# young-how/DQN-based-UAV-3D_path_planer

Hardware: NVIDIA H100
Metric: env steps/sec (+ DQN updates/sec), 500x500x100 city (higher is better)
Workload: dtype f64 env state / f32 obs+learner

## Files before the change

dqn-based-uav-3d_path_planer_b200/csrc/tc_forward.cu:

```cuda
#include "tc_forward.cuh"
#include "env_block.cuh"

#include <stdlib.h>
#include <string.h>

#include "tma.cuh"
#include "wgmma.cuh"

namespace uavrl {

static inline int rup(int x, int m) { return (x + m - 1) / m * m; }

size_t tc_smem_bytes(const TcNet &tc) { return (size_t)2 * tc.a_bytes + (size_t)tc.img_bytes + (size_t)tc.max_rows * tc.acc_ld * 4; }

int tc_build(const uavrl_learner_config &c, const NetDev &net, TcNet &tc, std::vector<int32_t> &hi_map, std::vector<int32_t> &lo_map,
             std::vector<int32_t> &hi2_map, std::vector<int32_t> &lo2_map)
{
    memset(&tc, 0, sizeof(tc));
    tc.n_layers = net.n_layers; tc.in_dim = net.in_dim; tc.n_actions = net.n_actions; tc.dueling = net.dueling;
    if (net.in_dim % 4 != 0) return -1;
    int off = 0, maxK = 0, k_pad = rup(net.in_dim, 8);
    for (int l = 0; l < net.n_layers; ++l) {
        const LayerDev &L = net.L[l];
        TcLayer &T = tc.L[l];
// ... 61 lines not shown
                if (l > 0) {
                    hi2_map[pi] = elem(T.N_pad, T.t_hi_off, k, o);
                    lo2_map[pi] = elem(T.N_pad, T.t_lo_off, k, o);
                }
            }
            hi_map[vrow ? (size_t)L.b2_off + (o - out_main) : (size_t)L.b_off + o] = tc.bias_base / 4 + T.bias_off + o;
        }
    }
    (void)c;
    return 0;
}


#define TC_TRACE(slot) do { if (a.trace && blockIdx.x == 0 && threadIdx.x == 0) a.trace[slot] = clock64(); } while (0)

template <bool FUSE_ENV, bool ACT, bool DUELING>
__global__ void __launch_bounds__(kTcThreads, 1) tc_forward_kernel_t(TcNet tc, TcArgs a, EnvFuse ef)
{
    TC_TRACE(0);
    extern __shared__ __align__(1024) unsigned char smem[];
    unsigned char *Ahi = smem, *Alo = smem + tc.a_bytes, *W = smem + 2 * tc.a_bytes;
    float *acc = reinterpret_cast<float *>(W + tc.img_bytes);
    __shared__ uint64_t wbar, wbar2;
    __shared__ const float *rows[kTcTile];
    __shared__ float s_rew[kTcTile], s_done[kTcTile];

    const int tid = threadIdx.x, warp = tid >> 5, lane = tid & 31, quad = warp & 3, half = warp >> 2;
    constexpr int kCtl = kTcThreads - 32;
    const bool early_w = (a.pdl & kPdlEarlyWeights) != 0;
    const uint32_t w_split = tc.n_layers > 1 ? (uint32_t)tc.L[1].hi_off : (uint32_t)tc.img_bytes;
    auto stage_image = [&]() {
// ... 72 lines not shown
            waited = true;
            if (tid == kCtl && !early_w) stage_image();
        }
        if (!wready) {
            __syncthreads();
            mbar_wait(&wbar, 0);
            wready = true;
        }
        TC_TRACE(3);
        fence_proxy_async();
        __syncthreads();
        TC_TRACE(4);

        for (int l = 0; l < tc.n_layers; ++l) {
            const TcLayer T = tc.L[l];
            mma_3xtf32(acc, tc.acc_ld, Ahi, Alo, W + T.hi_off, W + T.lo_off, mma_sbo(T.K_pad), T.N_pad, T.K_pad / 8, R);
            TC_TRACE(5 + 3 * l);
            if (!w2ready) { if (w_split < (uint32_t)tc.img_bytes) mbar_wait(&wbar2, 0); w2ready = true; }
            TC_TRACE(6 + 3 * l);
            const float *bias = bias_all + T.bias_off;
            const int row = quad * 32 + lane;
            const bool live = quad * 32 < R;
            if (l + 1 < tc.n_layers) {
                const uint32_t sbon = mma_sbo(T.N_pad);
                for (int c0 = half * 32; live && c0 < T.N_pad; c0 += 64) {
                    float v[32];
                    acc_ld32(acc, tc.acc_ld, row, c0, v);
#pragma unroll
                    for (int j = 0; j < 8; ++j) {
                        float4 h, lo4;
                        float x0 = fmaxf(v[4 * j + 0] + bias[c0 + 4 * j + 0], 0.f), x1 = fmaxf(v[4 * j + 1] + bias[c0 + 4 * j + 1], 0.f);
                        float x2 = fmaxf(v[4 * j + 2] + bias[c0 + 4 * j + 2], 0.f), x3 = fmaxf(v[4 * j + 3] + bias[c0 + 4 * j + 3], 0.f);
                        tf32_split(x0, h.x, lo4.x); tf32_split(x1, h.y, lo4.y); tf32_split(x2, h.z, lo4.z); tf32_split(x3, h.w, lo4.w);
                        const uint32_t off = mma_off(row, c0 + 4 * j, sbon);
                        *reinterpret_cast<float4 *>(Ahi + off) = h;
                        *reinterpret_cast<float4 *>(Alo + off) = lo4;
                    }
                }
                fence_proxy_async();
                __syncthreads();
                TC_TRACE(7 + 3 * l);
            } else {
                if (half == 0 && live) {
                    float q[32];
                    acc_ld32(acc, tc.acc_ld, row, 0, q);
                    const int nA = tc.n_actions;
#pragma unroll
                    for (int j = 0; j < 32; ++j) q[j] += bias[j];
                    if (DUELING) {
                        float s = 0.f;
#pragma unroll
                        for (int j = 0; j < 32; ++j) if (j < nA) s += q[j];
// ... 39 lines not shown
                }
                __syncthreads();
            }
        }
        if (FUSE_ENV) {
            __shared__ EnvSmem<32> env_sm;
            for (int sb = 0; sb < R; sb += 32)
                env_block<true, 32, kTcThreads, false, 8>(ef.d, env_sm, base + sb, tid, UAVRL_ACT_DISCRETE27, a.actions, ef.obs_next,
                                                       ef.reward, ef.done, nullptr, nullptr, nullptr);
            __syncthreads();
        }
    }
    TC_TRACE(20);
}

typedef void (*ForwardKernel)(TcNet, TcArgs, EnvFuse);
template <bool F, bool A>
static ForwardKernel pick_fwd_d(bool dueling) { return dueling ? tc_forward_kernel_t<F, A, true> : tc_forward_kernel_t<F, A, false>; }
static ForwardKernel pick_forward_kernel(bool fuse_env, bool act, bool dueling)
{
    if (fuse_env) return pick_fwd_d<true, true>(dueling);
    return act ? pick_fwd_d<false, true>(dueling) : pick_fwd_d<false, false>(dueling);
}

int launch_tc_forward(uavrl_learner *l, const TcArgs &a_in, cudaStream_t st, const EnvFuse *fuse)
{
    TcArgs a = a_in;
    const int n_sm = num_sms();
    a.rows_per_tile = (a.n >= 128 * n_sm && l->tc.max_rows == 128) ? 128 : (a.n >= 64 * n_sm) ? 64 : 32;
    a.n_tiles = (a.n + a.rows_per_tile - 1) / a.rows_per_tile;
    const int grid = a.n_tiles < n_sm ? a.n_tiles : n_sm;
    static const bool trace_on = getenv("UAVRL_TC_TRACE") != nullptr;
    long long *tr = nullptr;
    if (trace_on) { UAVRL_CUDA(cudaMalloc((void **)&tr, 32 * sizeof(long long))); UAVRL_CUDA(cudaMemset(tr, 0, 32 * sizeof(long long))); a.trace = tr; }
    const int prev = (l->pdl_chain && g_pdl.load()) ? l->pdl_prev : kPdlNone;
    a.pdl = 0;
    if (prev != kPdlNone) {
        a.pdl = kPdlOn;
        if (a.mode == kTcAct) {
            if (prev == kPdlAdam) a.pdl |= kPdlEarlyRows;
            else if (prev == kPdlEnv) a.pdl |= kPdlEarlyWeights;
        } else if (prev == kPdlEnv || prev == kPdlTd) {
            a.pdl |= kPdlEarlyWeights;
        }
    }
    EnvFuse ef;
    memset(&ef, 0, sizeof(ef));
    if (fuse) {
        ef = *fuse;
        UAVRL_CUDA(launch_kernel(pick_forward_kernel(true, a.mode == kTcAct, l->tc.dueling != 0), dim3(grid), dim3(kTcThreads), tc_smem_bytes(l->tc), st, a.pdl != 0, l->tc, a, ef));
        l->pdl_prev = l->pdl_chain ? kPdlEnv : kPdlNone;
    } else {
        UAVRL_CUDA(launch_kernel(pick_forward_kernel(false, a.mode == kTcAct, l->tc.dueling != 0), dim3(grid), dim3(kTcThreads), tc_smem_bytes(l->tc), st, a.pdl != 0, l->tc, a, ef));
        l->pdl_prev = l->pdl_chain ? (a.mode == kTcAct ? kPdlAct : kPdlTd) : kPdlNone;
    }
    UAVRL_LAUNCHED();
    if (trace_on) {
        long long h[32];
        UAVRL_CUDA(cudaStreamSynchronize(st));
        UAVRL_CUDA(cudaMemcpy(h, tr, sizeof(h), cudaMemcpyDeviceToHost));
        cudaFree(tr);
        fprintf(stderr, "[tc_trace] mode=%d n=%d R=%d grid=%d cycles since start:", a.mode, a.n, a.rows_per_tile, grid);
        for (int i = 1; i < 32; ++i) if (h[i]) fprintf(stderr, " [%d]=%lld", i, h[i] - h[0]);
        fprintf(stderr, "\n");
    }
    return 0;
}

// ... 5 lines not shown
    if (tc_smem_bytes(l->tc) > 227 * 1024) return 0;
    const size_t P = (size_t)l->net.P;
    const size_t img = (size_t)l->tc.train_img_bytes;
    UAVRL_CUDA(cudaMalloc((void **)&l->tc_img_local, img));
    UAVRL_CUDA(cudaMalloc((void **)&l->tc_img_target, img));
    UAVRL_CUDA(cudaMemset(l->tc_img_local, 0, img));
    UAVRL_CUDA(cudaMemset(l->tc_img_target, 0, img));
    int32_t **maps[] = { &l->tc_hi_map, &l->tc_lo_map, &l->tc_hi2_map, &l->tc_lo2_map };
    std::vector<int32_t> *src[] = { &hi, &lo, &hi2, &lo2 };
    for (int i = 0; i < 4; ++i) {
        UAVRL_CUDA(cudaMalloc((void **)maps[i], P * 4));
        UAVRL_CUDA(cudaMemcpy(*maps[i], src[i]->data(), P * 4, cudaMemcpyHostToDevice));
    }
    UAVRL_CUDA(cudaMalloc((void **)&l->y_buf, (size_t)l->cfg.batch_size * 4));
    UAVRL_CUDA(cudaMalloc((void **)&l->astar_buf, (size_t)l->cfg.batch_size * 4));
    for (int ac = 0; ac < 2; ++ac)
        for (int du = 0; du < 2; ++du)
            UAVRL_CUDA(cudaFuncSetAttribute(pick_forward_kernel(false, ac != 0, du != 0), cudaFuncAttributeMaxDynamicSharedMemorySize,
                                            (int)tc_smem_bytes(l->tc)));
    {
        l->fuse_ok = true;
        for (int du = 0; du < 2; ++du) {
            cudaFuncAttributes fa;
            UAVRL_CUDA(cudaFuncGetAttributes(&fa, pick_forward_kernel(true, true, du != 0)));
            if (fa.sharedSizeBytes + tc_smem_bytes(l->tc) > (size_t)227 * 1024) l->fuse_ok = false;
        }
        if (l->fuse_ok)
            for (int du = 0; du < 2; ++du)
                UAVRL_CUDA(cudaFuncSetAttribute(pick_forward_kernel(true, true, du != 0), cudaFuncAttributeMaxDynamicSharedMemorySize,
                                                (int)tc_smem_bytes(l->tc)));
    }
    l->y_cap = l->cfg.batch_size;
    l->tc_ok = true;
    return tc_train_init(l);
}

}
```

dqn-based-uav-3d_path_planer_b200/csrc/tc_forward.cuh:

```cuda
#pragma once
#include <vector>

#include "env.cuh"
#include "learner.cuh"

namespace uavrl {

constexpr int kTcThreads = 256;
constexpr int kTcTile = 128;

enum TcMode { kTcAct = 0, kTcArgmax = 1, kTcTdMax = 2, kTcTdGather = 3 };

struct TcArgs {
    const unsigned char *img;
    BatchSrc src;
    const float *obs;
    int32_t n, n_tiles, mode, use_next, rows_per_tile;
    float eps; int32_t is_train;
    const float *u_tape; const int32_t *rand_tape;
    uint64_t key, call;
    int32_t *actions;
    float *q_out;
    float *y_out;
    float gamma;
    int32_t pdl;
    long long *trace;
};

int tc_build(const uavrl_learner_config &c, const NetDev &net, TcNet &tc, std::vector<int32_t> &hi_map, std::vector<int32_t> &lo_map,
             std::vector<int32_t> &hi2_map, std::vector<int32_t> &lo2_map);
int tc_train_init(uavrl_learner *l);
int launch_tc_train(uavrl_learner *l, const BatchSrc &src, int B, int global_batch, const float *y, int *n_grad_parts,
                    int *n_loss_parts, cudaStream_t st, cudaEvent_t after_chain = nullptr, const AdamArgs *adam = nullptr,
                    float *loss_out = nullptr, bool *adam_done = nullptr, bool fused_td = false);
bool tc_train_can_fuse_td(const uavrl_learner *l, int B);
size_t tc_smem_bytes(const TcNet &tc);
struct EnvFuse { EnvDev d; float *obs_next; float *reward; uint8_t *done; };
int launch_tc_forward(uavrl_learner *l, const TcArgs &a, cudaStream_t st, const EnvFuse *fuse = nullptr);
int tc_init(uavrl_learner *l);

}
```

dqn-based-uav-3d_path_planer_b200/csrc/tc_train.cu:

```cuda
#include <string.h>
#include <stdlib.h>

#include <atomic>

#include "tc_forward.cuh"
#include "tma.cuh"
#include "wgmma.cuh"

namespace uavrl {

constexpr int kDwChunk = 128;

struct TcTrainArgs {
    const unsigned char *img;
    BatchSrc src;
    int32_t B, R, n_tiles;
    const float *y;
    float inv_global_b;
    float *act_buf, *dz_buf;
    float *loss_partials;
    int32_t loss_kind;
    int32_t fused_td, algo;
    float gamma;
    const unsigned char *img_target;
// ... 78 lines not shown
    for (int u = 0; u < 4; ++u) {
        const int i = threadIdx.x + u * kTcThreads;
        if (i < total) {
            const int r = i & (R - 1), j = i >> lgR;
            float4 h, l;
            tf32_split(v[u].x, h.x, l.x); tf32_split(v[u].y, h.y, l.y); tf32_split(v[u].z, h.z, l.z); tf32_split(v[u].w, h.w, l.w);
            const uint32_t off = mma_off(r, 4 * j, sbo);
            *reinterpret_cast<float4 *>(Ahi + off) = h;
            *reinterpret_cast<float4 *>(Alo + off) = l;
        }
    }
}

__device__ __forceinline__ uint32_t nl_split(const TcNet &tc) { return tc.n_layers > 1 ? (uint32_t)tc.L[1].hi_off : (uint32_t)tc.img_bytes; }

template <int NPRE, bool DUELING>
__global__ void __launch_bounds__(kTcThreads, 1) tc_train_kernel(TcNet tc, TcTrainArgs a)
{
    TR_TRACE(0);
    extern __shared__ __align__(1024) unsigned char smem[];
    const int R = a.R;
    const uint32_t a_bytes = (uint32_t)(R / 8) * mma_sbo(tc.max_k);
    unsigned char *Ahi = smem, *Alo = smem + a_bytes, *W = smem + 2 * a_bytes;
    float *acc = reinterpret_cast<float *>(W + tc.train_img_bytes);
    __shared__ uint64_t wbar, wbar2, wbar3;
    __shared__ const float *rows[kTcTile];
    __shared__ const float *rows2[kTcTile];
    __shared__ int s_act[kTcTile], s_astar[kTcTile];
    __shared__ uint8_t s_fresh[kTcTile];
    __shared__ float s_y[kTcTile], s_rew[kTcTile], s_done[kTcTile];
    __shared__ float s_loss;
// ... 13 lines not shown
            if (tc.train_img_bytes > tc.img_bytes)
                bulk_g2s_chunked(W + tc.img_bytes, a.img + tc.img_bytes, (uint32_t)(tc.train_img_bytes - tc.img_bytes), &wbar3);
        }
    }
    const uint32_t w_split = nl_split(tc);
    TR_TRACE(1);
    bool waited = false;
    const float *bias_all = reinterpret_cast<const float *>(W + tc.bias_base);

    uint32_t pkey[4];
    Philox::gen(a.src.key, a.src.epoch, 0x5A17ull, pkey);
    bool wready = false;
    const int nl = tc.n_layers;
    const int row = quad * 32 + lane;
    const bool live = quad * 32 < R;
    uint32_t hm1 = 0u, hm2 = 0u, hm3 = 0u, hm4 = 0u;

    for (int tile = blockIdx.x; tile < a.n_tiles; tile += gridDim.x) {
        const int base = tile * R;
        int64_t my_slot = -1;
        if (tid < R) {
            const int b = base + tid;
            const float *p = nullptr, *p2 = nullptr;
            bool fr = false;
            if (b < a.B) my_slot = resolve_rows(a.src, b, tc.in_dim, pkey, p, p2, &fr);
            rows[tid] = p;
            if (fused) { rows2[tid] = p2; s_astar[tid] = 0; s_fresh[tid] = fr ? 1 : 0; }
        }
        __syncthreads();
        const bool early_rows = n_pre > 0 && R * (tc.L[0].K_pad / 4) <= 4 * kTcThreads;
// ... 11 lines not shown
        for (int pass = 0; pass < n_pre; ++pass) {
            if (pass > 0 && tid == kTcThreads - 32) {
                fence_proxy_async();
                bulk_g2s_chunked(W, a.img_target, (uint32_t)tc.img_bytes, &wbar);
            }
            if (pass == 0 && early_rows) a0_store(vnext, R, tc.L[0].K_pad, Ahi, Alo);
            else build_a0(rows2, R, tc.in_dim, tc.L[0].K_pad, Ahi, Alo);
            if (pass == 0) { park_meta(); TR_TRACE(3); }
            mbar_wait(&wbar, wphase); wphase ^= 1;
            fence_proxy_async();
            __syncthreads();
            if (pass == 0) TR_TRACE(4);
            const bool td_pass = (pass == n_pre - 1);
            for (int l = 0; l < nl; ++l) {
                const TcLayer T = tc.L[l];
                mma_3xtf32(acc, tc.acc_ld, Ahi, Alo, W + T.hi_off, W + T.lo_off, mma_sbo(T.K_pad), T.N_pad, T.K_pad / 8, R);
                const float *bias = bias_all + T.bias_off;
                if (l + 1 < nl) {
                    const uint32_t sbon = mma_sbo(T.N_pad);
                    for (int c0 = half * 32; live && c0 < T.N_pad; c0 += 64) {
                        float v[32];
                        acc_ld32(acc, tc.acc_ld, row, c0, v);
#pragma unroll
                        for (int j = 0; j < 8; ++j) {
                            float4 x, h, lo4;
                            x.x = fmaxf(v[4 * j + 0] + bias[c0 + 4 * j + 0], 0.f); x.y = fmaxf(v[4 * j + 1] + bias[c0 + 4 * j + 1], 0.f);
                            x.z = fmaxf(v[4 * j + 2] + bias[c0 + 4 * j + 2], 0.f); x.w = fmaxf(v[4 * j + 3] + bias[c0 + 4 * j + 3], 0.f);
                            tf32_split(x.x, h.x, lo4.x); tf32_split(x.y, h.y, lo4.y); tf32_split(x.z, h.z, lo4.z); tf32_split(x.w, h.w, lo4.w);
                            const uint32_t off = mma_off(row, c0 + 4 * j, sbon);
                            *reinterpret_cast<float4 *>(Ahi + off) = h;
                            *reinterpret_cast<float4 *>(Alo + off) = lo4;
                        }
                    }
                } else if (half == 0 && live) {
                    float q[32];
                    acc_ld32(acc, tc.acc_ld, row, 0, q);
                    const int nA = tc.n_actions;
#pragma unroll
                    for (int j = 0; j < 32; ++j) q[j] += bias[j];
                    if (DUELING) {
                        float sA = 0.f, V = 0.f;
#pragma unroll
                        for (int j = 0; j < 32; ++j) { if (j < nA) sA += q[j]; if (j == nA) V = q[j]; }
                        const float mean = sA / (float)nA;
#pragma unroll
                        for (int j = 0; j < 32; ++j) q[j] = V + q[j] - mean;
                    }
// ... 23 lines not shown
            if (w_split < (uint32_t)tc.img_bytes) bulk_g2s_chunked(W + w_split, a.img + w_split, (uint32_t)tc.img_bytes - w_split, &wbar2);
        }
        if (early_rows) a0_store(vmain, R, tc.L[0].K_pad, Ahi, Alo);
        else build_a0(rows, R, tc.in_dim, tc.L[0].K_pad, Ahi, Alo);
        TR_TRACE(9);
        if (!waited) { pdl_wait(); pdl_trigger(); waited = true; }
        if (n_pre == 0) park_meta();
        if (!fused && tid < R) s_y[tid] = (base + tid < a.B) ? a.y[base + tid] : 0.f;
        if (fused) { mbar_wait(&wbar, wphase); wphase ^= 1; }
        else if (!wready) { mbar_wait(&wbar, 0); wready = true; }
        fence_proxy_async();
        __syncthreads();
        TR_TRACE(10);
        const int gb = base + row;
        const bool mine = live && gb < a.B;

        for (int l = 0; l < nl; ++l) {
            const TcLayer T = tc.L[l];
            mma_3xtf32(acc, tc.acc_ld, Ahi, Alo, W + T.hi_off, W + T.lo_off, mma_sbo(T.K_pad), T.N_pad, T.K_pad / 8, R);
            if (fused && l == 0 && w_split < (uint32_t)tc.img_bytes) mbar_wait(&wbar2, 0);
            if (l < 4) TR_TRACE(27 + l);
            const float *bias = bias_all + T.bias_off;
            if (l + 1 < nl) {
                const uint32_t sbon = mma_sbo(T.N_pad);
                float *act_row = a.act_buf + (size_t)gb * tc.act_stride + tc.L[l + 1].act_off;
                for (int c0 = half * 32; live && c0 < T.N_pad; c0 += 64) {
                    float v[32];
                    acc_ld32(acc, tc.acc_ld, row, c0, v);
                    uint32_t mk = 0u;
#pragma unroll
                    for (int j = 0; j < 8; ++j) {
                        float4 x, h, lo4;
                        x.x = fmaxf(v[4 * j + 0] + bias[c0 + 4 * j + 0], 0.f); x.y = fmaxf(v[4 * j + 1] + bias[c0 + 4 * j + 1], 0.f);
                        x.z = fmaxf(v[4 * j + 2] + bias[c0 + 4 * j + 2], 0.f); x.w = fmaxf(v[4 * j + 3] + bias[c0 + 4 * j + 3], 0.f);
                        tf32_split(x.x, h.x, lo4.x); tf32_split(x.y, h.y, lo4.y); tf32_split(x.z, h.z, lo4.z); tf32_split(x.w, h.w, lo4.w);
                        const uint32_t off = mma_off(row, c0 + 4 * j, sbon);
                        *reinterpret_cast<float4 *>(Ahi + off) = h;
                        *reinterpret_cast<float4 *>(Alo + off) = lo4;
                        if (mine) *reinterpret_cast<float4 *>(act_row + c0 + 4 * j) = x;
                        mk |= ((x.x > 0.f ? 1u : 0u) | (x.y > 0.f ? 2u : 0u) | (x.z > 0.f ? 4u : 0u) | (x.w > 0.f ? 8u : 0u)) << (4 * j);
                    }
                    if (!mine) mk = 0u;
                    if (l == 0) hm1 = mk; else if (l == 1) hm2 = mk; else if (l == 2) hm3 = mk; else hm4 = mk;
                }
            } else {
                const uint32_t sbon = mma_sbo(T.N_pad);
                if (half == 0 && live) {
                    float q[32];
                    acc_ld32(acc, tc.acc_ld, row, 0, q);
                    TR_TRACE(21);
                    const int nA = tc.n_actions;
#pragma unroll
                    for (int j = 0; j < 32; ++j) q[j] += bias[j];
                    if (DUELING) {
                        float s = 0.f, V = 0.f;
#pragma unroll
                        for (int j = 0; j < 32; ++j) { if (j < nA) s += q[j]; if (j == nA) V = q[j]; }
                        const float mean = s / (float)nA;
#pragma unroll
// ... 42 lines not shown
                        *reinterpret_cast<float4 *>(Ahi + off) = h;
                        *reinterpret_cast<float4 *>(Alo + off) = lo4;
                        if (mine) *reinterpret_cast<float4 *>(dz_row + 4 * j) = x;
                    }
                    TR_TRACE(26);
                }
            }
            fence_proxy_async();
            __syncthreads();
            TR_TRACE(11 + l);
        }

        if (fused && tc.train_img_bytes > tc.img_bytes) mbar_wait(&wbar3, 0);
        for (int l = nl - 1; l >= 1; --l) {
            const TcLayer T = tc.L[l];
            mma_3xtf32(acc, tc.acc_ld, Ahi, Alo, W + T.t_hi_off, W + T.t_lo_off, mma_sbo(T.N_pad), T.K_pad, T.N_pad / 8, R);
            const uint32_t hmask = (l == 1) ? hm1 : (l == 2) ? hm2 : (l == 3) ? hm3 : hm4;
            const uint32_t sbon = mma_sbo(T.K_pad);
            float *dz_row = a.dz_buf + (size_t)gb * tc.dz_stride + tc.L[l - 1].dz_off;
            {
                const int c0 = half * 32;
                if (live && c0 < T.K_pad) {
                    float v[32];
                    acc_ld32(acc, tc.acc_ld, row, c0, v);
#pragma unroll
                    for (int j = 0; j < 8; ++j) {
                        const uint32_t m4 = hmask >> (4 * j);
                        float4 x, h, lo4;
                        x.x = (m4 & 1u) ? v[4 * j + 0] : 0.f; x.y = (m4 & 2u) ? v[4 * j + 1] : 0.f;
                        x.z = (m4 & 4u) ? v[4 * j + 2] : 0.f; x.w = (m4 & 8u) ? v[4 * j + 3] : 0.f;
                        if (mine) *reinterpret_cast<float4 *>(dz_row + c0 + 4 * j) = x;
                        if (l > 1) {
                            tf32_split(x.x, h.x, lo4.x); tf32_split(x.y, h.y, lo4.y); tf32_split(x.z, h.z, lo4.z); tf32_split(x.w, h.w, lo4.w);
                            const uint32_t off = mma_off(row, c0 + 4 * j, sbon);
                            *reinterpret_cast<float4 *>(Ahi + off) = h;
                            *reinterpret_cast<float4 *>(Alo + off) = lo4;
                        }
                    }
                }
            }
            fence_proxy_async();
            __syncthreads();
            TR_TRACE(16 + l);
        }
    }
    TR_TRACE(20);
    if (tid == 0) a.loss_partials[blockIdx.x] = s_loss;
}

constexpr uint32_t kDwSbo = (kDwChunk / 4) * 128u + 16u;
constexpr int kDwARows = 128;

template <int LOG2F4, int U>
// ... 205 lines not shown
        }
        const float g = (g4[0] + g4[1]) + (g4[2] + g4[3]);
        a.ptrs.grad[i] = g;
        adam_update_one(a.adam, a.ptrs, i, g);
    }
    if (blockIdx.x == 0 && warp == 7 && a.ptrs.loss_out) {
        float sl = 0.f;
        for (int c = lane; c < a.adam.n_loss_parts; c += 32) sl += __ldcg(a.ptrs.loss_partials + c);
#pragma unroll
        for (int off = 16; off > 0; off >>= 1) sl += __shfl_xor_sync(0xffffffffu, sl, off);
        if (lane == 0) *a.ptrs.loss_out = sl * a.adam.inv_b;
    }
}

typedef void (*TrainKernel)(TcNet, TcTrainArgs);
template <int N>
static TrainKernel pick_train_d(bool dueling) { return dueling ? tc_train_kernel<N, true> : tc_train_kernel<N, false>; }
static TrainKernel pick_train_kernel(int npre, bool dueling) { return npre == 0 ? pick_train_d<0>(dueling) : npre == 1 ? pick_train_d<1>(dueling) : pick_train_d<2>(dueling); }

static size_t train_smem_bytes(const TcNet &tc, int R)
{
    return (size_t)2 * (R / 8) * mma_sbo(tc.max_k) + (size_t)tc.train_img_bytes + (size_t)R * tc.acc_ld * 4;
}
static size_t dw_smem_bytes(const TcNet &tc)
{
    int maxN = 32;
    for (int l = 0; l < tc.n_layers; ++l) if (tc.L[l].N_pad > maxN) maxN = tc.L[l].N_pad;
    return (size_t)2 * ((kDwARows + maxN) / 8) * kDwSbo;
}

int tc_train_init(uavrl_learner *l)
{
    l->tc_train_ok = false;
    const TcNet &tc = l->tc;
    for (int i = 0; i < tc.n_layers; ++i)
        if (tc.L[i].K_real + 1 > 128 || tc.L[i].K_real % 4 != 0 || (tc.L[i].N_pad != 32 && tc.L[i].N_pad != 64)) return 0;
    if (train_smem_bytes(tc, 32) > 227 * 1024 || dw_smem_bytes(tc) > 227 * 1024) return 0;
    if (train_smem_bytes(tc, 32) < (size_t)(32 / 8) * mma_sbo(tc.max_k) + (size_t)8 * mma_sbo(tc.max_k)) return 0;
    for (int np = 0; np < 3; ++np)
        for (int du = 0; du < 2; ++du)
            UAVRL_CUDA(cudaFuncSetAttribute(pick_train_kernel(np, du != 0), cudaFuncAttributeMaxDynamicSharedMemorySize,
                                            (int)(train_smem_bytes(tc, 64) <= 227 * 1024 ? train_smem_bytes(tc, 64) : train_smem_bytes(tc, 32))));
    UAVRL_CUDA(cudaFuncSetAttribute(tc_dw_kernel<false>, cudaFuncAttributeMaxDynamicSharedMemorySize, (int)dw_smem_bytes(tc)));
    UAVRL_CUDA(cudaFuncSetAttribute(tc_dw_kernel<true>, cudaFuncAttributeMaxDynamicSharedMemorySize, (int)dw_smem_bytes(tc)));
    const size_t cap = (size_t)l->cfg.batch_size;
    UAVRL_CUDA(cudaMalloc((void **)&l->act_buf, cap * (size_t)(tc.act_stride > 0 ? tc.act_stride : 4) * 4));
    UAVRL_CUDA(cudaMalloc((void **)&l->dz_buf, cap * (size_t)tc.dz_stride * 4));
    l->train_cap = (int32_t)cap;
    l->tc_train_ok = true;
    return 0;
}

std::atomic<int> g_fuse_td{1};
static int train_rows_per_tile(const TcNet &tc, int B)
{
    return (B > 32 * num_sms() && train_smem_bytes(tc, 64) <= 227 * 1024) ? 64 : 32;
// ... 15 lines not shown
    memset(&a, 0, sizeof(a));
    a.img = l->tc_img_local; a.src = src; a.B = B; a.y = y; a.inv_global_b = 1.0f / (float)global_batch;
    a.act_buf = l->act_buf; a.dz_buf = l->dz_buf; a.loss_partials = l->loss_partials;
    a.loss_kind = l->cfg.loss_kind;
    a.fused_td = fused_td ? 1 : 0; a.algo = l->cfg.algo; a.gamma = l->cfg.gamma; a.img_target = l->tc_img_target;
    a.R = train_rows_per_tile(tc, B);
    a.n_tiles = (B + a.R - 1) / a.R;
    const int grid = a.n_tiles < num_sms() ? a.n_tiles : num_sms();
    const bool chain = l->pdl_chain && g_pdl.load();
    if (fused_td && a.n_tiles > grid) return fail(UAVRL_ERR_INVALID, "fused TD needs one tile per CTA");
    static const bool trace_on = getenv("UAVRL_TC_TRACE") != nullptr;
    long long *tr = nullptr;
    if (trace_on) { UAVRL_CUDA(cudaMalloc((void **)&tr, 48 * sizeof(long long))); UAVRL_CUDA(cudaMemset(tr, 0, 48 * sizeof(long long))); a.trace = tr + 16; }
    const bool use_pdl = chain && (fused_td ? (l->pdl_prev == kPdlEnv) : (l->pdl_prev == kPdlTd));
    const int npre = fused_td ? (l->cfg.algo != UAVRL_ALGO_DQN ? 2 : 1) : 0;
    auto train_fn = pick_train_kernel(npre, tc.dueling != 0);
    UAVRL_CUDA(launch_kernel(train_fn, dim3(grid), dim3(kTcThreads), train_smem_bytes(tc, a.R), st, use_pdl, tc, a));
    static const bool twice = trace_on && getenv("UAVRL_TRAIN_TWICE") != nullptr;
    if (twice) UAVRL_CUDA(launch_kernel(train_fn, dim3(grid), dim3(kTcThreads), train_smem_bytes(tc, a.R), st, false, tc, a));
    l->pdl_prev = chain ? kPdlTrain : kPdlNone;
    UAVRL_LAUNCHED();
    if (after_chain) UAVRL_CUDA(cudaEventRecord(after_chain, st));
    TcDwArgs d;
    memset(&d, 0, sizeof(d));
    d.src = src; d.B = B; d.n_chunks = (B + kDwChunk - 1) / kDwChunk; d.P = l->net.P;
    d.act_buf = l->act_buf; d.dz_buf = l->dz_buf; d.partials = l->partials;
    const int n_sm = num_sms();
    const int max_slices = n_sm / tc.n_layers > 0 ? n_sm / tc.n_layers : 1;
    d.n_slices = d.n_chunks < max_slices ? d.n_chunks : max_slices;
    const int dw_grid = d.n_slices * tc.n_layers;
    const bool fuse = adam != nullptr && g_fuse_dw_adam.load() && dw_grid <= n_sm;
// ... 46 lines not shown
```

dqn-based-uav-3d_path_planer_b200/csrc/wgmma.cuh:

```cuda
#pragma once
#include <stdint.h>

namespace uavrl {

constexpr uint32_t kMmaLBO = 128;

__host__ __device__ constexpr uint32_t mma_sbo(int k_pad) { return (uint32_t)(k_pad / 4) * 128u; }
__host__ __device__ constexpr uint32_t mma_tile_bytes(int rows, int k_pad) { return (uint32_t)(rows / 8) * mma_sbo(k_pad); }

__device__ __forceinline__ uint32_t mma_off(int r, int c, uint32_t sbo, uint32_t lbo = kMmaLBO)
{
    return (uint32_t)(r >> 3) * sbo + (uint32_t)(c >> 2) * lbo + (uint32_t)(r & 7) * 16u + (uint32_t)(c & 3) * 4u;
}

__device__ __forceinline__ uint64_t mma_desc(const void *smem_ptr, uint32_t sbo, uint32_t lbo = kMmaLBO)
{
    const uint32_t addr = (uint32_t)__cvta_generic_to_shared(smem_ptr);
    uint64_t d = 0;
    d |= (uint64_t)((addr >> 4) & 0x3FFFu);
    d |= (uint64_t)((lbo >> 4) & 0x3FFFu) << 16;
    d |= (uint64_t)((sbo >> 4) & 0x3FFFu) << 32;
    return d;
}

// ... 39 lines not shown
template <int N>
__device__ __forceinline__ void wgmma_3xtf32(float *d, uint64_t a_hi, uint64_t a_lo, uint64_t b_hi, uint64_t b_lo, int ksteps,
                                             uint32_t accumulate)
{
    const uint64_t kStep = (uint64_t)((2 * kMmaLBO) >> 4);
    fence_operands<N>(d);
    wgmma_fence();
    for (int k = 0; k < ksteps; ++k) wgmma_tf32<N>(d, a_hi + k * kStep, b_hi + k * kStep, (k > 0 || accumulate) ? 1u : 0u);
    for (int k = 0; k < ksteps; ++k) wgmma_tf32<N>(d, a_hi + k * kStep, b_lo + k * kStep, 1u);
    for (int k = 0; k < ksteps; ++k) wgmma_tf32<N>(d, a_lo + k * kStep, b_hi + k * kStep, 1u);
    wgmma_commit();
    wgmma_wait0();
    fence_operands<N>(d);
}

template <int N>
__device__ __forceinline__ void store_frag(const float *d, float *acc, int ld, int row0, int col0, int R)
{
    const int t = threadIdx.x & 127, r = row0 + 16 * (t >> 5) + ((t & 31) >> 2), c = col0 + 2 * (t & 3);
#pragma unroll
    for (int i = 0; i < N / 8; ++i) {
        if (r < R) *reinterpret_cast<float2 *>(acc + (size_t)r * ld + c + 8 * i) = make_float2(d[4 * i], d[4 * i + 1]);
        if (r + 8 < R) *reinterpret_cast<float2 *>(acc + (size_t)(r + 8) * ld + c + 8 * i) = make_float2(d[4 * i + 2], d[4 * i + 3]);
    }
}

template <int N>
__device__ __forceinline__ void mma_chunk(float *acc, int ld, int row0, int n0, uint64_t a_hi, uint64_t a_lo, const unsigned char *b_hi,
                                          const unsigned char *b_lo, uint32_t sbo, int ksteps, int R)
{
    float d[N / 2];
    const uint32_t boff = (uint32_t)(n0 >> 3) * sbo;
    wgmma_3xtf32<N>(d, a_hi, a_lo, mma_desc(b_hi + boff, sbo), mma_desc(b_lo + boff, sbo), ksteps, 0u);
    store_frag<N>(d, acc, ld, row0, n0, R);
}

__device__ __forceinline__ void mma_3xtf32(float *acc, int ld, const unsigned char *a_hi, const unsigned char *a_lo,
                                           const unsigned char *b_hi, const unsigned char *b_lo, uint32_t sbo, int N, int ksteps, int R)
{
    const int row0 = (threadIdx.x >> 7) * 64;
    if (row0 < R) {
        const uint64_t ah = mma_desc(a_hi + (row0 >> 3) * sbo, sbo), al = mma_desc(a_lo + (row0 >> 3) * sbo, sbo);
        int n0 = 0;
        for (; n0 + 64 <= N; n0 += 64) mma_chunk<64>(acc, ld, row0, n0, ah, al, b_hi, b_lo, sbo, ksteps, R);
        if (n0 + 32 <= N) { mma_chunk<32>(acc, ld, row0, n0, ah, al, b_hi, b_lo, sbo, ksteps, R); n0 += 32; }
        if (n0 < N) mma_chunk<16>(acc, ld, row0, n0, ah, al, b_hi, b_lo, sbo, ksteps, R);
    }
    __syncthreads();
}

__device__ __forceinline__ void acc_ld32(const float *acc, int ld, int row, int c0, float (&v)[32])
{
    const float4 *src = reinterpret_cast<const float4 *>(acc + (size_t)row * ld + c0);
#pragma unroll
    for (int j = 0; j < 8; ++j) {
        const float4 t = src[j];
        v[4 * j] = t.x; v[4 * j + 1] = t.y; v[4 * j + 2] = t.z; v[4 * j + 3] = t.w;
    }
}

}
```

Baseline: 70.60 million.

## Specialize wgmma k-loops for fixed shapes and redistribute epilogue work across all threads

```diff
diff --git a/dqn-based-uav-3d_path_planer_b200/csrc/tc_forward.cu b/dqn-based-uav-3d_path_planer_b200/csrc/tc_forward.cu
--- a/dqn-based-uav-3d_path_planer_b200/csrc/tc_forward.cu
+++ b/dqn-based-uav-3d_path_planer_b200/csrc/tc_forward.cu
@@ -99,7 +99,7 @@
 
 #define TC_TRACE(slot) do { if (a.trace && blockIdx.x == 0 && threadIdx.x == 0) a.trace[slot] = clock64(); } while (0)
 
-template <bool FUSE_ENV, bool ACT, bool DUELING>
+template <bool FUSE_ENV, bool ACT, bool DUELING, bool FIXED>
 __global__ void __launch_bounds__(kTcThreads, 1) tc_forward_kernel_t(TcNet tc, TcArgs a, EnvFuse ef)
 {
     TC_TRACE(0);
@@ -202,7 +202,7 @@
 
         for (int l = 0; l < tc.n_layers; ++l) {
             const TcLayer T = tc.L[l];
-            mma_3xtf32(acc, tc.acc_ld, Ahi, Alo, W + T.hi_off, W + T.lo_off, mma_sbo(T.K_pad), T.N_pad, T.K_pad / 8, R);
+            mma_3xtf32<kMmaFwd, FIXED>(acc, tc.acc_ld, Ahi, Alo, W + T.hi_off, W + T.lo_off, mma_sbo(T.K_pad), T.N_pad, T.K_pad / 8, R);
             TC_TRACE(5 + 3 * l);
             if (!w2ready) { if (w_split < (uint32_t)tc.img_bytes) mbar_wait(&wbar2, 0); w2ready = true; }
             TC_TRACE(6 + 3 * l);
@@ -211,19 +211,16 @@
             const bool live = quad * 32 < R;
             if (l + 1 < tc.n_layers) {
                 const uint32_t sbon = mma_sbo(T.N_pad);
-                for (int c0 = half * 32; live && c0 < T.N_pad; c0 += 64) {
-                    float v[32];
-                    acc_ld32(acc, tc.acc_ld, row, c0, v);
-#pragma unroll
-                    for (int j = 0; j < 8; ++j) {
-                        float4 h, lo4;
-                        float x0 = fmaxf(v[4 * j + 0] + bias[c0 + 4 * j + 0], 0.f), x1 = fmaxf(v[4 * j + 1] + bias[c0 + 4 * j + 1], 0.f);
-                        float x2 = fmaxf(v[4 * j + 2] + bias[c0 + 4 * j + 2], 0.f), x3 = fmaxf(v[4 * j + 3] + bias[c0 + 4 * j + 3], 0.f);
-                        tf32_split(x0, h.x, lo4.x); tf32_split(x1, h.y, lo4.y); tf32_split(x2, h.z, lo4.z); tf32_split(x3, h.w, lo4.w);
-                        const uint32_t off = mma_off(row, c0 + 4 * j, sbon);
-                        *reinterpret_cast<float4 *>(Ahi + off) = h;
-                        *reinterpret_cast<float4 *>(Alo + off) = lo4;
-                    }
+                const EpiSlice e(R, kTcThreads);
+                for (int c = e.c0; c < T.N_pad; c += e.step) {
+                    const float4 v = e.ld(acc, tc.acc_ld, c);
+                    float4 h, lo4;
+                    const float x0 = fmaxf(v.x + bias[c + 0], 0.f), x1 = fmaxf(v.y + bias[c + 1], 0.f);
+                    const float x2 = fmaxf(v.z + bias[c + 2], 0.f), x3 = fmaxf(v.w + bias[c + 3], 0.f);
+                    tf32_split(x0, h.x, lo4.x); tf32_split(x1, h.y, lo4.y); tf32_split(x2, h.z, lo4.z); tf32_split(x3, h.w, lo4.w);
+                    const uint32_t off = mma_off(e.row, c, sbon);
+                    *reinterpret_cast<float4 *>(Ahi + off) = h;
+                    *reinterpret_cast<float4 *>(Alo + off) = lo4;
                 }
                 fence_proxy_async();
                 __syncthreads();
@@ -293,13 +290,25 @@
     TC_TRACE(20);
 }
 
+bool tc_fixed_chains(const TcNet &tc, bool train)
+{
+    for (int l = 0; l < tc.n_layers; ++l) {
+        const TcLayer &T = tc.L[l];
+        if (!mma_fixed_product(kMmaFwd, T.N_pad, T.K_pad / 8)) return false;
+        if (train && l > 0 && !mma_fixed_product(kMmaDx, T.K_pad, T.N_pad / 8)) return false;
+    }
+    return true;
+}
+
 typedef void (*ForwardKernel)(TcNet, TcArgs, EnvFuse);
+template <bool F, bool A, bool D>
+static ForwardKernel pick_fwd_x(bool fixed) { return fixed ? tc_forward_kernel_t<F, A, D, true> : tc_forward_kernel_t<F, A, D, false>; }
 template <bool F, bool A>
-static ForwardKernel pick_fwd_d(bool dueling) { return dueling ? tc_forward_kernel_t<F, A, true> : tc_forward_kernel_t<F, A, false>; }
-static ForwardKernel pick_forward_kernel(bool fuse_env, bool act, bool dueling)
-{
-    if (fuse_env) return pick_fwd_d<true, true>(dueling);
-    return act ? pick_fwd_d<false, true>(dueling) : pick_fwd_d<false, false>(dueling);
+static ForwardKernel pick_fwd_d(bool dueling, bool fixed) { return dueling ? pick_fwd_x<F, A, true>(fixed) : pick_fwd_x<F, A, false>(fixed); }
+static ForwardKernel pick_forward_kernel(bool fuse_env, bool act, bool dueling, bool fixed)
+{
+    if (fuse_env) return pick_fwd_d<true, true>(dueling, fixed);
+    return act ? pick_fwd_d<false, true>(dueling, fixed) : pick_fwd_d<false, false>(dueling, fixed);
 }
 
 int launch_tc_forward(uavrl_learner *l, const TcArgs &a_in, cudaStream_t st, const EnvFuse *fuse)
@@ -327,10 +336,10 @@
     memset(&ef, 0, sizeof(ef));
     if (fuse) {
         ef = *fuse;
-        UAVRL_CUDA(launch_kernel(pick_forward_kernel(true, a.mode == kTcAct, l->tc.dueling != 0), dim3(grid), dim3(kTcThreads), tc_smem_bytes(l->tc), st, a.pdl != 0, l->tc, a, ef));
+        UAVRL_CUDA(launch_kernel(pick_forward_kernel(true, a.mode == kTcAct, l->tc.dueling != 0, tc_fixed_chains(l->tc, false)), dim3(grid), dim3(kTcThreads), tc_smem_bytes(l->tc), st, a.pdl != 0, l->tc, a, ef));
         l->pdl_prev = l->pdl_chain ? kPdlEnv : kPdlNone;
     } else {
-        UAVRL_CUDA(launch_kernel(pick_forward_kernel(false, a.mode == kTcAct, l->tc.dueling != 0), dim3(grid), dim3(kTcThreads), tc_smem_bytes(l->tc), st, a.pdl != 0, l->tc, a, ef));
+        UAVRL_CUDA(launch_kernel(pick_forward_kernel(false, a.mode == kTcAct, l->tc.dueling != 0, tc_fixed_chains(l->tc, false)), dim3(grid), dim3(kTcThreads), tc_smem_bytes(l->tc), st, a.pdl != 0, l->tc, a, ef));
         l->pdl_prev = l->pdl_chain ? (a.mode == kTcAct ? kPdlAct : kPdlTd) : kPdlNone;
     }
     UAVRL_LAUNCHED();
@@ -366,20 +375,21 @@
     }
     UAVRL_CUDA(cudaMalloc((void **)&l->y_buf, (size_t)l->cfg.batch_size * 4));
     UAVRL_CUDA(cudaMalloc((void **)&l->astar_buf, (size_t)l->cfg.batch_size * 4));
+    const bool fixed = tc_fixed_chains(l->tc, false);
     for (int ac = 0; ac < 2; ++ac)
         for (int du = 0; du < 2; ++du)
-            UAVRL_CUDA(cudaFuncSetAttribute(pick_forward_kernel(false, ac != 0, du != 0), cudaFuncAttributeMaxDynamicSharedMemorySize,
+            UAVRL_CUDA(cudaFuncSetAttribute(pick_forward_kernel(false, ac != 0, du != 0, fixed), cudaFuncAttributeMaxDynamicSharedMemorySize,
                                             (int)tc_smem_bytes(l->tc)));
     {
         l->fuse_ok = true;
         for (int du = 0; du < 2; ++du) {
             cudaFuncAttributes fa;
-            UAVRL_CUDA(cudaFuncGetAttributes(&fa, pick_forward_kernel(true, true, du != 0)));
+            UAVRL_CUDA(cudaFuncGetAttributes(&fa, pick_forward_kernel(true, true, du != 0, fixed)));
             if (fa.sharedSizeBytes + tc_smem_bytes(l->tc) > (size_t)227 * 1024) l->fuse_ok = false;
         }
         if (l->fuse_ok)
             for (int du = 0; du < 2; ++du)
-                UAVRL_CUDA(cudaFuncSetAttribute(pick_forward_kernel(true, true, du != 0), cudaFuncAttributeMaxDynamicSharedMemorySize,
+                UAVRL_CUDA(cudaFuncSetAttribute(pick_forward_kernel(true, true, du != 0, fixed), cudaFuncAttributeMaxDynamicSharedMemorySize,
                                                 (int)tc_smem_bytes(l->tc)));
     }
     l->y_cap = l->cfg.batch_size;
diff --git a/dqn-based-uav-3d_path_planer_b200/csrc/tc_forward.cuh b/dqn-based-uav-3d_path_planer_b200/csrc/tc_forward.cuh
--- a/dqn-based-uav-3d_path_planer_b200/csrc/tc_forward.cuh
+++ b/dqn-based-uav-3d_path_planer_b200/csrc/tc_forward.cuh
@@ -35,6 +35,7 @@
                     float *loss_out = nullptr, bool *adam_done = nullptr, bool fused_td = false);
 bool tc_train_can_fuse_td(const uavrl_learner *l, int B);
 size_t tc_smem_bytes(const TcNet &tc);
+bool tc_fixed_chains(const TcNet &tc, bool train);
 struct EnvFuse { EnvDev d; float *obs_next; float *reward; uint8_t *done; };
 int launch_tc_forward(uavrl_learner *l, const TcArgs &a, cudaStream_t st, const EnvFuse *fuse = nullptr);
 int tc_init(uavrl_learner *l);
diff --git a/dqn-based-uav-3d_path_planer_b200/csrc/tc_train.cu b/dqn-based-uav-3d_path_planer_b200/csrc/tc_train.cu
--- a/dqn-based-uav-3d_path_planer_b200/csrc/tc_train.cu
+++ b/dqn-based-uav-3d_path_planer_b200/csrc/tc_train.cu
@@ -116,7 +116,7 @@
 
 __device__ __forceinline__ uint32_t nl_split(const TcNet &tc) { return tc.n_layers > 1 ? (uint32_t)tc.L[1].hi_off : (uint32_t)tc.img_bytes; }
 
-template <int NPRE, bool DUELING>
+template <int NPRE, bool DUELING, bool FIXED>
 __global__ void __launch_bounds__(kTcThreads, 1) tc_train_kernel(TcNet tc, TcTrainArgs a)
 {
     TR_TRACE(0);
@@ -160,6 +160,7 @@
     const int nl = tc.n_layers;
     const int row = quad * 32 + lane;
     const bool live = quad * 32 < R;
+    const EpiSlice e(R, kTcThreads);
     uint32_t hm1 = 0u, hm2 = 0u, hm3 = 0u, hm4 = 0u;
 
     for (int tile = blockIdx.x; tile < a.n_tiles; tile += gridDim.x) {
@@ -201,23 +202,19 @@
             const bool td_pass = (pass == n_pre - 1);
             for (int l = 0; l < nl; ++l) {
                 const TcLayer T = tc.L[l];
-                mma_3xtf32(acc, tc.acc_ld, Ahi, Alo, W + T.hi_off, W + T.lo_off, mma_sbo(T.K_pad), T.N_pad, T.K_pad / 8, R);
+                mma_3xtf32<kMmaFwd, FIXED>(acc, tc.acc_ld, Ahi, Alo, W + T.hi_off, W + T.lo_off, mma_sbo(T.K_pad), T.N_pad, T.K_pad / 8, R);
                 const float *bias = bias_all + T.bias_off;
                 if (l + 1 < nl) {
                     const uint32_t sbon = mma_sbo(T.N_pad);
-                    for (int c0 = half * 32; live && c0 < T.N_pad; c0 += 64) {
-                        float v[32];
-                        acc_ld32(acc, tc.acc_ld, row, c0, v);
-#pragma unroll
-                        for (int j = 0; j < 8; ++j) {
-                            float4 x, h, lo4;
-                            x.x = fmaxf(v[4 * j + 0] + bias[c0 + 4 * j + 0], 0.f); x.y = fmaxf(v[4 * j + 1] + bias[c0 + 4 * j + 1], 0.f);
-                            x.z = fmaxf(v[4 * j + 2] + bias[c0 + 4 * j + 2], 0.f); x.w = fmaxf(v[4 * j + 3] + bias[c0 + 4 * j + 3], 0.f);
-                            tf32_split(x.x, h.x, lo4.x); tf32_split(x.y, h.y, lo4.y); tf32_split(x.z, h.z, lo4.z); tf32_split(x.w, h.w, lo4.w);
-                            const uint32_t off = mma_off(row, c0 + 4 * j, sbon);
-                            *reinterpret_cast<float4 *>(Ahi + off) = h;
-                            *reinterpret_cast<float4 *>(Alo + off) = lo4;
-                        }
+                    for (int c = e.c0; c < T.N_pad; c += e.step) {
+                        const float4 v = e.ld(acc, tc.acc_ld, c);
+                        float4 x, h, lo4;
+                        x.x = fmaxf(v.x + bias[c + 0], 0.f); x.y = fmaxf(v.y + bias[c + 1], 0.f);
+                        x.z = fmaxf(v.z + bias[c + 2], 0.f); x.w = fmaxf(v.w + bias[c + 3], 0.f);
+                        tf32_split(x.x, h.x, lo4.x); tf32_split(x.y, h.y, lo4.y); tf32_split(x.z, h.z, lo4.z); tf32_split(x.w, h.w, lo4.w);
+                        const uint32_t off = mma_off(e.row, c, sbon);
+                        *reinterpret_cast<float4 *>(Ahi + off) = h;
+                        *reinterpret_cast<float4 *>(Alo + off) = lo4;
                     }
                 } else if (half == 0 && live) {
                     float q[32];
@@ -271,35 +268,33 @@
         TR_TRACE(10);
         const int gb = base + row;
         const bool mine = live && gb < a.B;
+        const int egb = base + e.row;
+        const bool emine = egb < a.B;
 
         for (int l = 0; l < nl; ++l) {
             const TcLayer T = tc.L[l];
-            mma_3xtf32(acc, tc.acc_ld, Ahi, Alo, W + T.hi_off, W + T.lo_off, mma_sbo(T.K_pad), T.N_pad, T.K_pad / 8, R);
+            mma_3xtf32<kMmaFwd, FIXED>(acc, tc.acc_ld, Ahi, Alo, W + T.hi_off, W + T.lo_off, mma_sbo(T.K_pad), T.N_pad, T.K_pad / 8, R);
             if (fused && l == 0 && w_split < (uint32_t)tc.img_bytes) mbar_wait(&wbar2, 0);
             if (l < 4) TR_TRACE(27 + l);
             const float *bias = bias_all + T.bias_off;
             if (l + 1 < nl) {
                 const uint32_t sbon = mma_sbo(T.N_pad);
-                float *act_row = a.act_buf + (size_t)gb * tc.act_stride + tc.L[l + 1].act_off;
-                for (int c0 = half * 32; live && c0 < T.N_pad; c0 += 64) {
-                    float v[32];
-                    acc_ld32(acc, tc.acc_ld, row, c0, v);
-                    uint32_t mk = 0u;
-#pragma unroll
-                    for (int j = 0; j < 8; ++j) {
-                        float4 x, h, lo4;
-                        x.x = fmaxf(v[4 * j + 0] + bias[c0 + 4 * j + 0], 0.f); x.y = fmaxf(v[4 * j + 1] + bias[c0 + 4 * j + 1], 0.f);
-                        x.z = fmaxf(v[4 * j + 2] + bias[c0 + 4 * j + 2], 0.f); x.w = fmaxf(v[4 * j + 3] + bias[c0 + 4 * j + 3], 0.f);
-                        tf32_split(x.x, h.x, lo4.x); tf32_split(x.y, h.y, lo4.y); tf32_split(x.z, h.z, lo4.z); tf32_split(x.w, h.w, lo4.w);
-                        const uint32_t off = mma_off(row, c0 + 4 * j, sbon);
-                        *reinterpret_cast<float4 *>(Ahi + off) = h;
-                        *reinterpret_cast<float4 *>(Alo + off) = lo4;
-                        if (mine) *reinterpret_cast<float4 *>(act_row + c0 + 4 * j) = x;
-                        mk |= ((x.x > 0.f ? 1u : 0u) | (x.y > 0.f ? 2u : 0u) | (x.z > 0.f ? 4u : 0u) | (x.w > 0.f ? 8u : 0u)) << (4 * j);
-                    }
-                    if (!mine) mk = 0u;
-                    if (l == 0) hm1 = mk; else if (l == 1) hm2 = mk; else if (l == 2) hm3 = mk; else hm4 = mk;
+                float *act_row = a.act_buf + (size_t)egb * tc.act_stride + tc.L[l + 1].act_off;
+                uint32_t mk = 0u;
+                for (int c = e.c0, sh = 0; c < T.N_pad; c += e.step, sh += 4) {
+                    const float4 v = e.ld(acc, tc.acc_ld, c);
+                    float4 x, h, lo4;
+                    x.x = fmaxf(v.x + bias[c + 0], 0.f); x.y = fmaxf(v.y + bias[c + 1], 0.f);
+                    x.z = fmaxf(v.z + bias[c + 2], 0.f); x.w = fmaxf(v.w + bias[c + 3], 0.f);
+                    tf32_split(x.x, h.x, lo4.x); tf32_split(x.y, h.y, lo4.y); tf32_split(x.z, h.z, lo4.z); tf32_split(x.w, h.w, lo4.w);
+                    const uint32_t off = mma_off(e.row, c, sbon);
+                    *reinterpret_cast<float4 *>(Ahi + off) = h;
+                    *reinterpret_cast<float4 *>(Alo + off) = lo4;
+                    if (emine) *reinterpret_cast<float4 *>(act_row + c) = x;
+                    mk |= ((x.x > 0.f ? 1u : 0u) | (x.y > 0.f ? 2u : 0u) | (x.z > 0.f ? 4u : 0u) | (x.w > 0.f ? 8u : 0u)) << sh;
                 }
+                if (!emine) mk = 0u;
+                if (l == 0) hm1 = mk; else if (l == 1) hm2 = mk; else if (l == 2) hm3 = mk; else hm4 = mk;
             } else {
                 const uint32_t sbon = mma_sbo(T.N_pad);
                 if (half == 0 && live) {
@@ -372,29 +367,22 @@
         if (fused && tc.train_img_bytes > tc.img_bytes) mbar_wait(&wbar3, 0);
         for (int l = nl - 1; l >= 1; --l) {
             const TcLayer T = tc.L[l];
-            mma_3xtf32(acc, tc.acc_ld, Ahi, Alo, W + T.t_hi_off, W + T.t_lo_off, mma_sbo(T.N_pad), T.K_pad, T.N_pad / 8, R);
+            mma_3xtf32<kMmaDx, FIXED>(acc, tc.acc_ld, Ahi, Alo, W + T.t_hi_off, W + T.t_lo_off, mma_sbo(T.N_pad), T.K_pad, T.N_pad / 8, R);
             const uint32_t hmask = (l == 1) ? hm1 : (l == 2) ? hm2 : (l == 3) ? hm3 : hm4;
             const uint32_t sbon = mma_sbo(T.K_pad);
-            float *dz_row = a.dz_buf + (size_t)gb * tc.dz_stride + tc.L[l - 1].dz_off;
-            {
-                const int c0 = half * 32;
-                if (live && c0 < T.K_pad) {
-                    float v[32];
-                    acc_ld32(acc, tc.acc_ld, row, c0, v);
-#pragma unroll
-                    for (int j = 0; j < 8; ++j) {
-                        const uint32_t m4 = hmask >> (4 * j);
-                        float4 x, h, lo4;
-                        x.x = (m4 & 1u) ? v[4 * j + 0] : 0.f; x.y = (m4 & 2u) ? v[4 * j + 1] : 0.f;
-                        x.z = (m4 & 4u) ? v[4 * j + 2] : 0.f; x.w = (m4 & 8u) ? v[4 * j + 3] : 0.f;
-                        if (mine) *reinterpret_cast<float4 *>(dz_row + c0 + 4 * j) = x;
-                        if (l > 1) {
-                            tf32_split(x.x, h.x, lo4.x); tf32_split(x.y, h.y, lo4.y); tf32_split(x.z, h.z, lo4.z); tf32_split(x.w, h.w, lo4.w);
-                            const uint32_t off = mma_off(row, c0 + 4 * j, sbon);
-                            *reinterpret_cast<float4 *>(Ahi + off) = h;
-                            *reinterpret_cast<float4 *>(Alo + off) = lo4;
-                        }
-                    }
+            float *dz_row = a.dz_buf + (size_t)egb * tc.dz_stride + tc.L[l - 1].dz_off;
+            for (int c = e.c0, sh = 0; c < T.K_pad; c += e.step, sh += 4) {
+                const float4 v = e.ld(acc, tc.acc_ld, c);
+                const uint32_t m4 = hmask >> sh;
+                float4 x, h, lo4;
+                x.x = (m4 & 1u) ? v.x : 0.f; x.y = (m4 & 2u) ? v.y : 0.f;
+                x.z = (m4 & 4u) ? v.z : 0.f; x.w = (m4 & 8u) ? v.w : 0.f;
+                if (emine) *reinterpret_cast<float4 *>(dz_row + c) = x;
+                if (l > 1) {
+                    tf32_split(x.x, h.x, lo4.x); tf32_split(x.y, h.y, lo4.y); tf32_split(x.z, h.z, lo4.z); tf32_split(x.w, h.w, lo4.w);
+                    const uint32_t off = mma_off(e.row, c, sbon);
+                    *reinterpret_cast<float4 *>(Ahi + off) = h;
+                    *reinterpret_cast<float4 *>(Alo + off) = lo4;
                 }
             }
             fence_proxy_async();
@@ -630,9 +618,14 @@
 }
 
 typedef void (*TrainKernel)(TcNet, TcTrainArgs);
+template <int N, bool D>
+static TrainKernel pick_train_x(bool fixed) { return fixed ? tc_train_kernel<N, D, true> : tc_train_kernel<N, D, false>; }
 template <int N>
-static TrainKernel pick_train_d(bool dueling) { return dueling ? tc_train_kernel<N, true> : tc_train_kernel<N, false>; }
-static TrainKernel pick_train_kernel(int npre, bool dueling) { return npre == 0 ? pick_train_d<0>(dueling) : npre == 1 ? pick_train_d<1>(dueling) : pick_train_d<2>(dueling); }
+static TrainKernel pick_train_d(bool dueling, bool fixed) { return dueling ? pick_train_x<N, true>(fixed) : pick_train_x<N, false>(fixed); }
+static TrainKernel pick_train_kernel(int npre, bool dueling, bool fixed)
+{
+    return npre == 0 ? pick_train_d<0>(dueling, fixed) : npre == 1 ? pick_train_d<1>(dueling, fixed) : pick_train_d<2>(dueling, fixed);
+}
 
 static size_t train_smem_bytes(const TcNet &tc, int R)
 {
@@ -655,7 +648,7 @@
     if (train_smem_bytes(tc, 32) < (size_t)(32 / 8) * mma_sbo(tc.max_k) + (size_t)8 * mma_sbo(tc.max_k)) return 0;
     for (int np = 0; np < 3; ++np)
         for (int du = 0; du < 2; ++du)
-            UAVRL_CUDA(cudaFuncSetAttribute(pick_train_kernel(np, du != 0), cudaFuncAttributeMaxDynamicSharedMemorySize,
+            UAVRL_CUDA(cudaFuncSetAttribute(pick_train_kernel(np, du != 0, tc_fixed_chains(tc, true)), cudaFuncAttributeMaxDynamicSharedMemorySize,
                                             (int)(train_smem_bytes(tc, 64) <= 227 * 1024 ? train_smem_bytes(tc, 64) : train_smem_bytes(tc, 32))));
     UAVRL_CUDA(cudaFuncSetAttribute(tc_dw_kernel<false>, cudaFuncAttributeMaxDynamicSharedMemorySize, (int)dw_smem_bytes(tc)));
     UAVRL_CUDA(cudaFuncSetAttribute(tc_dw_kernel<true>, cudaFuncAttributeMaxDynamicSharedMemorySize, (int)dw_smem_bytes(tc)));
@@ -701,7 +694,7 @@
     if (trace_on) { UAVRL_CUDA(cudaMalloc((void **)&tr, 48 * sizeof(long long))); UAVRL_CUDA(cudaMemset(tr, 0, 48 * sizeof(long long))); a.trace = tr + 16; }
     const bool use_pdl = chain && (fused_td ? (l->pdl_prev == kPdlEnv) : (l->pdl_prev == kPdlTd));
     const int npre = fused_td ? (l->cfg.algo != UAVRL_ALGO_DQN ? 2 : 1) : 0;
-    auto train_fn = pick_train_kernel(npre, tc.dueling != 0);
+    auto train_fn = pick_train_kernel(npre, tc.dueling != 0, tc_fixed_chains(tc, true));
     UAVRL_CUDA(launch_kernel(train_fn, dim3(grid), dim3(kTcThreads), train_smem_bytes(tc, a.R), st, use_pdl, tc, a));
     static const bool twice = trace_on && getenv("UAVRL_TRAIN_TWICE") != nullptr;
     if (twice) UAVRL_CUDA(launch_kernel(train_fn, dim3(grid), dim3(kTcThreads), train_smem_bytes(tc, a.R), st, false, tc, a));
diff --git a/dqn-based-uav-3d_path_planer_b200/csrc/wgmma.cuh b/dqn-based-uav-3d_path_planer_b200/csrc/wgmma.cuh
--- a/dqn-based-uav-3d_path_planer_b200/csrc/wgmma.cuh
+++ b/dqn-based-uav-3d_path_planer_b200/csrc/wgmma.cuh
@@ -77,6 +77,44 @@
     fence_operands<N>(d);
 }
 
+template <int N, int KS>
+__device__ __forceinline__ void wgmma_3xtf32_k(float *d, uint64_t a_hi, uint64_t a_lo, uint64_t b_hi, uint64_t b_lo)
+{
+    const uint64_t kStep = (uint64_t)((2 * kMmaLBO) >> 4);
+    fence_operands<N>(d);
+    wgmma_fence();
+#pragma unroll
+    for (int k = 0; k < KS; ++k) wgmma_tf32<N>(d, a_hi + k * kStep, b_hi + k * kStep, k > 0 ? 1u : 0u);
+#pragma unroll
+    for (int k = 0; k < KS; ++k) wgmma_tf32<N>(d, a_hi + k * kStep, b_lo + k * kStep, 1u);
+#pragma unroll
+    for (int k = 0; k < KS; ++k) wgmma_tf32<N>(d, a_lo + k * kStep, b_hi + k * kStep, 1u);
+    wgmma_commit();
+    wgmma_wait0();
+    fence_operands<N>(d);
+}
+
+enum MmaKind { kMmaFwd = 0, kMmaDx = 1 };
+
+__host__ __device__ constexpr bool mma_fixed(int kind, int n, int ksteps)
+{
+    return kind == kMmaFwd ? (n == 64 && (ksteps == 13 || ksteps == 8 || ksteps == 16)) || (n == 32 && ksteps == 8)
+                           : n == 64 && (ksteps == 4 || ksteps == 8);
+}
+__host__ __device__ constexpr bool mma_fixed_product(int kind, int n, int ksteps)
+{
+    return (n < 64 || mma_fixed(kind, 64, ksteps)) && (n % 64 < 32 || mma_fixed(kind, 32, ksteps)) && n % 32 == 0;
+}
+
+template <int N, int KIND>
+__device__ __forceinline__ void wgmma_3xtf32_fixed(float *d, uint64_t a_hi, uint64_t a_lo, uint64_t b_hi, uint64_t b_lo, int ksteps)
+{
+    if constexpr (mma_fixed(KIND, N, 4)) if (ksteps == 4) wgmma_3xtf32_k<N, 4>(d, a_hi, a_lo, b_hi, b_lo);
+    if constexpr (mma_fixed(KIND, N, 8)) if (ksteps == 8) wgmma_3xtf32_k<N, 8>(d, a_hi, a_lo, b_hi, b_lo);
+    if constexpr (mma_fixed(KIND, N, 13)) if (ksteps == 13) wgmma_3xtf32_k<N, 13>(d, a_hi, a_lo, b_hi, b_lo);
+    if constexpr (mma_fixed(KIND, N, 16)) if (ksteps == 16) wgmma_3xtf32_k<N, 16>(d, a_hi, a_lo, b_hi, b_lo);
+}
+
 template <int N>
 __device__ __forceinline__ void store_frag(const float *d, float *acc, int ld, int row0, int col0, int R)
 {
@@ -88,16 +126,19 @@
     }
 }
 
-template <int N>
+template <int N, int KIND, bool FIXED>
 __device__ __forceinline__ void mma_chunk(float *acc, int ld, int row0, int n0, uint64_t a_hi, uint64_t a_lo, const unsigned char *b_hi,
                                           const unsigned char *b_lo, uint32_t sbo, int ksteps, int R)
 {
     float d[N / 2];
     const uint32_t boff = (uint32_t)(n0 >> 3) * sbo;
-    wgmma_3xtf32<N>(d, a_hi, a_lo, mma_desc(b_hi + boff, sbo), mma_desc(b_lo + boff, sbo), ksteps, 0u);
+    const uint64_t bh = mma_desc(b_hi + boff, sbo), bl = mma_desc(b_lo + boff, sbo);
+    if (FIXED) wgmma_3xtf32_fixed<N, KIND>(d, a_hi, a_lo, bh, bl, ksteps);
+    else wgmma_3xtf32<N>(d, a_hi, a_lo, bh, bl, ksteps, 0u);
     store_frag<N>(d, acc, ld, row0, n0, R);
 }
 
+template <int KIND, bool FIXED>
 __device__ __forceinline__ void mma_3xtf32(float *acc, int ld, const unsigned char *a_hi, const unsigned char *a_lo,
                                            const unsigned char *b_hi, const unsigned char *b_lo, uint32_t sbo, int N, int ksteps, int R)
 {
@@ -105,9 +146,9 @@
     if (row0 < R) {
         const uint64_t ah = mma_desc(a_hi + (row0 >> 3) * sbo, sbo), al = mma_desc(a_lo + (row0 >> 3) * sbo, sbo);
         int n0 = 0;
-        for (; n0 + 64 <= N; n0 += 64) mma_chunk<64>(acc, ld, row0, n0, ah, al, b_hi, b_lo, sbo, ksteps, R);
-        if (n0 + 32 <= N) { mma_chunk<32>(acc, ld, row0, n0, ah, al, b_hi, b_lo, sbo, ksteps, R); n0 += 32; }
-        if (n0 < N) mma_chunk<16>(acc, ld, row0, n0, ah, al, b_hi, b_lo, sbo, ksteps, R);
+        for (; n0 + 64 <= N; n0 += 64) mma_chunk<64, KIND, FIXED>(acc, ld, row0, n0, ah, al, b_hi, b_lo, sbo, ksteps, R);
+        if (n0 + 32 <= N) { mma_chunk<32, KIND, FIXED>(acc, ld, row0, n0, ah, al, b_hi, b_lo, sbo, ksteps, R); n0 += 32; }
+        if (!FIXED && n0 < N) mma_chunk<16, KIND, FIXED>(acc, ld, row0, n0, ah, al, b_hi, b_lo, sbo, ksteps, R);
     }
     __syncthreads();
 }
@@ -122,4 +163,17 @@
     }
 }
 
+struct EpiSlice {
+    int row, c0, step;
+    __device__ __forceinline__ EpiSlice(int R, int nt)
+    {
+        const int lgR = 31 - __clz(R);
+        row = threadIdx.x & (R - 1); c0 = 4 * (threadIdx.x >> lgR); step = 4 * (nt >> lgR);
+    }
+    __device__ __forceinline__ float4 ld(const float *acc, int ld, int c) const
+    {
+        return *reinterpret_cast<const float4 *>(acc + (size_t)row * ld + c);
+    }
+};
+
 }
```

Result: faster. 76.38 million, median of 6 (+8.2%).
